# TigreGotico/phoonnx

Hardware: AMD Instinct MI355X
Metric: audio samples/sec (22.05 kHz), batch-32 256-phoneme utterances (higher is better)
Workload: dtype f32 (f16x3 split: fp32 operands as two fp16 planes, three MFMA products, fp32 accumulate)

## Files before the change

include/vitsmi.h:

```cpp
#ifndef VITSMI_H
#define VITSMI_H

#include <stddef.h>
#include <stdint.h>

#ifdef __cplusplus
extern "C" {
#endif

typedef struct vits_handle vits_handle;

enum {
    VITS_OK = 0,
    VITS_E_IO = -1,
    VITS_E_FORMAT = -2,
    VITS_E_ARG = -3,
    VITS_E_DEVICE = -4,
    VITS_E_NOMEM = -5,
    VITS_E_RANGE = -6
};

#define VITS_MAX_DIMS 4


// ... 418 lines not shown
    int res_planes;
    float res_slope;
    const float *old_out;
    const float *bias_b;
    int bias_b_stride;
    float div, oslope, oslope2, islope;
    const int64_t *lens;
    int rag_add, rag_mul;
    float sentinel;
    float *out;
    float *planes_out;
    float *res_seen;
    char kernel[128];
    int pack_cfg, run_cfg_used, rawin, s16, ck;
    float peak;
} vits_test_conv_sx_epi_args;
int vits_test_conv1d_sx_epi(int device_id, vits_test_conv_sx_epi_args *a);
int vits_test_conv1d_sx_planar(int device_id, const float *x, int B, int Cin, int T, const float *w, const float *bias,
                               int Cout, int K, int dil, int flags, const int64_t *lens, const float *old, int row_split,
                               int pl_rows, float *out, float *planes_out);
long long vits_test_set_sx_small_max(long long wgs);
int vits_test_conv1d_sx_gate(int device_id, const float *x, int B, int Cin, int T, const float *w, const float *bias,
                             const float *bias_b, int Cout, int K, int dil, int flags, float *out);
int vits_test_conv_transpose1d_sx(int device_id, const float *x, int B, int Cin, int T, const float *w,
                                  const float *bias, int Cout, int K, int stride, float *out);
int vits_bench_conv1d_sx(int device_id, int B, int Cin, int Cout, int T, int K, int dil, int dbg, int iters,
                         float *ms_out);
int vits_test_conv_pair_sx(int device_id, const float *x, int B, int C, int T, const float *w1, const float *b1,
                           const float *w2, const float *b2, int K, int dil1, int dil2, int chain, float slope, float *out,
                           float *ms_out);
// ... 1 lines not shown
typedef struct {
    int B, C, T, K, dil1, dil2, chain;
    int flags;
    float slope, div;
    const float *x;
    const float *w1, *b1, *w2, *b2;
    const int64_t *lens;
    const float *out_init;
    float *out;
    char kernel[128];
    int BNo;
} vits_test_conv_pair_sx_epi_args;
int vits_test_conv_pair_sx_epi(int device_id, vits_test_conv_pair_sx_epi_args *a);
int vits_test_split_identity(const float *x, int64_t n, uint16_t *h1_old, uint16_t *h1_fused);
int64_t vits_test_split_identity_sweep(uint32_t first, uint64_t count, uint32_t *first_bad);
int vits_test_split_forms(int device_id, const float *x, int n, float slope, int form, uint16_t *h0, uint16_t *h1, float *pk,
                          float *rec);
enum { VITS_P16_EPI_ACC = 1, VITS_P16_EPI_DIV = 2, VITS_P16_EPI_RAW = 4, VITS_P16_EPI_PLANES = 8 };
typedef struct {
    int B, C, T, K, dil1, dil2, chain;
    int precision;
    int flags;
    float slope, div, sentinel;
    const float *x;
    const float *w1, *b1, *w2, *b2;
    const float *old_out;
    const float *x_tail;
    const int64_t *lens;
    int rag_add, rag_mul;
    float *out;
// ... 139 lines not shown
```

phoonnx_amd/_ffi.py:

```python
import ctypes as C
import os

import numpy as np

from . import audio_encoding

_HERE = os.path.dirname(os.path.abspath(__file__))
_LIB = None

VITS_MAX_DIMS = 4


class VitsNoise(C.Structure):
    _fields_ = [("noise_dp", C.c_void_p), ("noise_z", C.c_void_p), ("noise_z_stride", C.c_int64),
                ("seed", C.c_uint64)]


class VitsOutput(C.Structure):
    _fields_ = [("data", C.POINTER(C.c_float)), ("dims", C.c_int64 * 4), ("y_lengths", C.POINTER(C.c_int64))]


class VitsStats(C.Structure):
    _fields_ = [("conv_flops", C.c_double), ("conv_bytes", C.c_double), ("dec_flops", C.c_double),
                ("dec_bytes", C.c_double), ("flow_flops", C.c_double), ("enc_flops", C.c_double),
# ... 15 lines not shown
               [(n, C.c_void_p) for n in ("x", "w", "bias", "lens", "bias_b")] + [("bias_b_stride", C.c_int), ("res", C.c_void_p)] + \
               [(n, C.c_int) for n in ("x_cstride", "out_cstride", "out_rows", "out_row0")] + \
               [("old_out", C.c_void_p), ("old_out2", C.c_void_p), ("sentinel", C.c_float), ("out", C.c_void_p), ("out2", C.c_void_p),
                ("pl_rows", C.c_int), ("planes_out", C.c_void_p), ("kernel", C.c_char * 128), ("cfg_used", C.c_int), ("ck_used", C.c_int)]


class VitsTestConvSxEpiArgs(C.Structure):
    _fields_ = [(n, C.c_int) for n in ("B", "Cin", "T", "Cout", "K", "dil", "pad_l", "stride", "precision", "force16", "no_s16",
                                       "min_cfg", "run_cfg", "flags")] + \
               [(n, C.c_void_p) for n in ("x", "w", "bias", "res")] + \
               [("res_is_x", C.c_int), ("res_planes", C.c_int), ("res_slope", C.c_float), ("old_out", C.c_void_p),
                ("bias_b", C.c_void_p), ("bias_b_stride", C.c_int)] + \
               [(n, C.c_float) for n in ("div", "oslope", "oslope2", "islope")] + \
               [("lens", C.c_void_p), ("rag_add", C.c_int), ("rag_mul", C.c_int), ("sentinel", C.c_float), ("out", C.c_void_p),
                ("planes_out", C.c_void_p), ("res_seen", C.c_void_p), ("kernel", C.c_char * 128)] + \
               [(n, C.c_int) for n in ("pack_cfg", "run_cfg_used", "rawin", "s16", "ck")] + [("peak", C.c_float)]


class VitsTestConvPair16EpiArgs(C.Structure):
    _fields_ = [(n, C.c_int) for n in ("B", "C", "T", "K", "dil1", "dil2", "chain", "precision", "flags")] + \
               [(n, C.c_float) for n in ("slope", "div", "sentinel")] + \
               [(n, C.c_void_p) for n in ("x", "w1", "b1", "w2", "b2", "old_out", "x_tail", "lens")] + \
               [("rag_add", C.c_int), ("rag_mul", C.c_int)] + \
               [(n, C.c_void_p) for n in ("out", "planes_out", "x_seen", "ms_out")] + [("kernel", C.c_char * 128)] + \
               [(n, C.c_int) for n in ("BN", "BNo", "ovl")] + [("peak", C.c_float), ("guard_ok", C.c_int)]


class VitsTestConvPairSxEpiArgs(C.Structure):
    _fields_ = [(n, C.c_int) for n in ("B", "C", "T", "K", "dil1", "dil2", "chain", "flags")] + \
               [(n, C.c_float) for n in ("slope", "div")] + \
               [(n, C.c_void_p) for n in ("x", "w1", "b1", "w2", "b2", "lens", "out_init", "out")] + \
# ... 133 lines not shown
    "vits_test_durations", "vits_test_expand_prior", "vits_test_fill_normal", "vits_test_fill_normal_rows", "vits_test_post_conv",
    "vits_delivery_plan", "vits_deliver", "vits_test_deliver",
    "vits_trim_range", "vits_delivery_plan_trimmed", "vits_deliver_trimmed", "vits_test_deliver_trimmed",
    "vits_loudness_filter", "vits_loudness_gate", "vits_level_gain", "vits_delivery_plan_leveled", "vits_deliver_leveled",
    "vits_test_loudness_blocks", "vits_test_deliver_leveled",
    "vits_shape_check", "vits_shape_gain", "vits_deliver_shaped", "vits_test_deliver_shaped",
    "vits_limit_check", "vits_limit_gains", "vits_deliver_limited", "vits_test_deliver_limited",
    "vits_run_chunked_enc", "vits_run_vocoder_chunked_enc", "vits_test_stream_pack",
    "vits_stream_shaping_check", "vits_stream_emit_range", "vits_run_chunked_enc_shaped", "vits_run_vocoder_chunked_enc_shaped",
    "vits_test_stream_pack_shaped",
    "vits_stream_onset_check", "vits_stream_onset_start", "vits_run_chunked_enc_trimmed", "vits_run_vocoder_chunked_enc_trimmed",
    "vits_test_stream_pack_trimmed",
    "vits_test_layernorm", "vits_test_dds", "vits_test_cf_pre", "vits_test_rqs_inverse", "vits_test_ea_logw",
    "vits_test_conv1d_epi", "vits_test_wn_gate", "vits_test_cond_matvec", "vits_test_conv1d_sx_epi",
    "vits_test_conv_pair16_epi", "vits_test_attention_form", "vits_test_conv_pair_sx_epi", "vits_test_split_forms", "vits_test_split_identity", "vits_test_split_identity_sweep",
]


G2P_EXPORTS = ["g2p_open", "g2p_close", "g2p_last_error", "g2p_hparam", "g2p_num_outputs", "g2p_output_name", "g2p_bucket",
               "g2p_run", "g2p_generate", "g2p_generate_batch", "g2p_test_forced_steps", "g2p_test_linear", "g2p_test_step"]


def lib_path():
    return os.environ.get("VITSMI_LIB") or os.path.join(_HERE, "libvitsmi.so")


def load():
    global _LIB
    if _LIB is not None:
        return _LIB
# ... 194 lines not shown
    lib.vits_test_conv1d_sx.argtypes = lib.vits_test_conv1d.argtypes
    lib.vits_test_conv_transpose1d_sx.argtypes = lib.vits_test_conv_transpose1d.argtypes
    lib.vits_test_conv1d_sx_planar.argtypes = [C.c_int, vp, C.c_int, C.c_int, C.c_int, vp, vp, C.c_int, C.c_int, C.c_int, C.c_int,
                                               vp, vp, C.c_int, C.c_int, vp, vp]
    lib.vits_test_set_sx_small_max.argtypes = [C.c_longlong]
    lib.vits_test_set_sx_small_max.restype = C.c_longlong
    lib.vits_test_conv1d_sx_gate.argtypes = [C.c_int, vp, C.c_int, C.c_int, C.c_int, vp, vp, vp, C.c_int, C.c_int, C.c_int, C.c_int, vp]
    lib.vits_bench_conv1d_sx.argtypes = [C.c_int] * 9 + [f32p]
    lib.vits_test_conv1d_epi.argtypes = [C.c_int, C.POINTER(VitsTestConvEpiArgs)]
    lib.vits_test_conv1d_sx_epi.argtypes = [C.c_int, C.POINTER(VitsTestConvSxEpiArgs)]
    lib.vits_test_conv_pair16_epi.argtypes = [C.c_int, C.POINTER(VitsTestConvPair16EpiArgs)]
    lib.vits_test_conv_pair_sx_epi.argtypes = [C.c_int, C.POINTER(VitsTestConvPairSxEpiArgs)]
    lib.vits_test_split_identity.argtypes = [vp, C.c_int64, vp, vp]
    lib.vits_test_split_identity_sweep.argtypes = [C.c_uint32, C.c_uint64, C.POINTER(C.c_uint32)]
    lib.vits_test_split_identity_sweep.restype = C.c_int64
    lib.vits_test_split_forms.argtypes = [C.c_int, vp, C.c_int, C.c_float, C.c_int, vp, vp, vp, vp]
    lib.vits_test_attention_form.argtypes = [C.c_int, C.POINTER(VitsTestAttentionFormArgs)]
    lib.vits_test_wn_gate.argtypes = [C.c_int, vp, C.c_int, C.c_int, C.c_int, C.c_int, vp]
    lib.vits_test_cond_matvec.argtypes = [C.c_int, vp, C.c_int, C.c_int, vp, C.c_int, vp, vp, C.c_int, vp]
    lib.vits_test_conv_pair_sx.argtypes = [C.c_int, vp, C.c_int, C.c_int, C.c_int, vp, vp, vp, vp, C.c_int, C.c_int,
                                           C.c_int, C.c_int, C.c_float, vp, f32p]
    lib.g2p_open.argtypes = [C.c_char_p, C.c_int, C.POINTER(vp)]
    lib.g2p_close.argtypes = [vp]
    lib.g2p_close.restype = None
    lib.g2p_last_error.argtypes = [vp]
    lib.g2p_last_error.restype = C.c_char_p
    lib.g2p_hparam.argtypes = [vp, C.c_char_p, i64p]
    lib.g2p_num_outputs.argtypes = [vp]
    lib.g2p_output_name.argtypes = [vp, C.c_int]
    lib.g2p_output_name.restype = C.c_char_p
# ... 18 lines not shown
```

phoonnx_amd/csrc/conv_sx_engine.hip.hpp:

```cpp
#pragma once
#include <hip/hip_runtime.h>
#include <stdint.h>

#include <cstdio>
#include <cstdlib>
#include <string>
#include <utility>

#include "conv_engine.hip.hpp"
#include "conv_geom.hpp"

#ifndef SX_CFG0_WIDE
#define SX_CFG0_WIDE 0
#endif
#ifndef SX16_SPREAD
#define SX16_SPREAD 0
#endif
#ifndef SX16_PRIO
#define SX16_PRIO 0
#endif
#ifndef SX16_ABL
#define SX16_ABL 0
#endif
#ifndef SX16_NA_SMALL
#define SX16_NA_SMALL 2
#endif
#ifndef SX16_WIDE
#define SX16_WIDE 1
#endif
#ifndef SX_NOA
#define SX_NOA 0
#endif
#ifndef SX_XCD_GROUP_DEFAULT
#define SX_XCD_GROUP_DEFAULT 4
#endif
namespace vitsmi {

typedef __bf16 bf16x8 __attribute__((ext_vector_type(8)));
typedef _Float16 f16x8 __attribute__((ext_vector_type(8)));

enum : int { SX_NO_RAW_STORE = 256 };

struct SxRagged {
    const int *len;
    int add, mul;
};
// ... 33 lines not shown
    int64_t planar_bstride;
    int RS;
    int s16;
    unsigned magic;
    unsigned x_bytes;
    unsigned lds_bytes;
    int NT, MT, B;
    int flags;
    float div, oslope, oslope2;
    float wscale;
    unsigned long long *prof;
    unsigned *peak;
    SxRagged rag;
    int zt_p = -1;
    int xgs = 0;
};

inline int sx_xcd_group_shift() {
    static const int v = [] {
        const char *e = std::getenv("VITSMI_XCD_GROUP");
        int g = e ? std::atoi(e) : SX_XCD_GROUP_DEFAULT, s = 0;
        while ((2 << s) <= g && s < 4) s++;
        return s;
    }();
    return v;
}
__device__ __forceinline__ int sx_xcd_tile(int tseq, int xcd, int xgs) {
    return ((tseq >> xgs) << (xgs + 3)) + (xcd << xgs) + (tseq & ((1 << xgs) - 1));
}

// ... 88 lines not shown
}

__device__ __forceinline__ float f16_bits_to_f32(unsigned short h) { return (float)__builtin_bit_cast(_Float16, h); }

enum : int {
    SX_HAS_RAW = 1 << 9,
    SX_HAS_PL = 1 << 10,
    SX_RAW_ACT = 1 << 11,
    SX_PL_ACT = 1 << 12,
    SX_HAS_BIASB = 1 << 13,
    SX_RES_EARLY = 1 << 14,
    SX_GATE = 1 << 15,
    SX_WN_RMW = 1 << 19,
    SX_PLANAR_STORE2 = 1 << 20,
    SX_PLANAR_COUPLING = 1 << 21,
    SX_RES_PL = 1 << 22
};
constexpr int kSxEpiMask = EPI_RES | EPI_ACC | EPI_DIV | SX_HAS_RAW | SX_HAS_PL | SX_RAW_ACT | SX_PL_ACT | SX_HAS_BIASB | SX_RES_EARLY |
                           SX_GATE | SX_RES_PL;

template <int MW, int NW, int WM, int WN, int EPI = -1, bool PROF = false, bool RAWIN = false, int NP = 6, int SH = 32>
__global__ __launch_bounds__(256, (MW * NW > 8) ? 1 : ((SH == 16 && MW * NW == 2 && !RAWIN) ? 3 : 2)) void conv_sx_kernel(SxArgs a) {
    constexpr int BM = MW * WM * 32, BN = NW * WN * 32, MB = BM / 32;
    constexpr bool S16 = SH == 16;
    static_assert(SH == 32 || (SH == 16 && (NP == 2 || NP == 1) && !RAWIN && !PROF), "16x16x32: fp16 arithmetics on plane inputs");
    static_assert(NP == 6 || NP == 1 || NP == 2, "arithmetic");
    static_assert(NP != 1 || SH == 16, "the single-plane mode exists on the 16x16x32 loop only");
    constexpr bool H1 = NP == 1;
    constexpr bool F16 = NP == 2 || H1;
    constexpr int NPROD = H1 ? 1 : (F16 ? 3 : NP);
    constexpr int NPL = NP == 6 ? 3 : (H1 ? 1 : 2);
// ... 737 lines not shown
    const float *resb = a.res + (int64_t)b * a.raw_bstride;
    const uint16_t *resplb = a.res_pl + (int64_t)b * a.pl_bstride;
    const float unsl = a.res_unslope;
    const bool respl = H1 || (EPI >= 0 ? (EPI & SX_RES_PL) != 0 : a.res_pl != nullptr);
    const bool res_epi = (flags & EPI_RES) && !PRE;
    const float *addp = res_epi ? resb : rawb;
    const bool has_add = res_epi || (flags & EPI_ACC);
    const bool two_adds = res_epi && (flags & EPI_ACC);
    const float oslope = a.oslope, oslope2 = a.oslope2, rdiv = a.div;
    const float wsc = a.wscale;
    const int64_t plane_elems = (int64_t)CGo * Tout * 8;
    const float *biasp = a.bias ? a.bias : a.zeros;
    const int b_on = a.bias ? 1 : 0;
    constexpr int NRND = MW * (NW / 2);
    constexpr bool PIPE = EPI >= 0 && ((EPI & EPI_RES) != 0 && !PRE) != ((EPI & EPI_ACC) != 0);
    f32x4 adb[PIPE ? 2 : 1][2][4], ad2[2][4];
    auto geom = [&](int m, int n, int &co0, int &r, int &t) {
        const int row0 = mt * BM + (wm * MW + m) * 32;
        r = u == 1 ? 0 : (row0 >> 5) % u;
        co0 = u == 1 ? row0 : (row0 / (32 * u)) * 32;
        t = t0 + (wn * NW + n) * 32 + l31;
    };
    auto cell_at = [&](int co0, int r, int t, int q) -> int64_t {
        return ((int64_t)((co0 >> 3) + q) * Tout + (t * u + r)) * 8 + 4 * hi;
    };
    auto issue_adds = [&](auto R, auto P) {
        constexpr int rr = decltype(R)::value, pp = decltype(P)::value;
        constexpr int m = rr / (NW / 2), n0 = (rr % (NW / 2)) * 2;
#pragma unroll
        for (int j = 0; j < 2; j++) {
            int co0, r, t;
            geom(m, n0 + j, co0, r, t);
            const int tl = t < T ? t : T - 1;
#pragma unroll
            for (int q = 0; q < 4; q++) {
                const int64_t c = cell_at(co0, r, tl, q);
                if (respl) {
                    if (res_epi) {
                        float o4[4];
                        if constexpr (H1) {
                            unact4h(*reinterpret_cast<const u32x2 *>(resplb + c), unsl, o4);
                        } else {
                            float h0[4], h1[4];
                            unact4h(*reinterpret_cast<const u32x2 *>(resplb + c), 1.f, h0);
                            unact4h(*reinterpret_cast<const u32x2 *>(resplb + plane_elems + c), 1.f, h1);
#pragma unroll
                            for (int e = 0; e < 4; e++) {
// ... 24 lines not shown
        const int row0 = mt * BM + (wm * MW + m) * 32;
        f32x4 bq[4];
#pragma unroll
        for (int q = 0; q < 4; q++) {
            bq[q] = *reinterpret_cast<const f32x4 *>(biasp + (row0 + 8 * q + 4 * hi) * b_on);
            if (flags & SX_HAS_BIASB)
                bq[q] += *reinterpret_cast<const f32x4 *>(a.bias_b + (int64_t)b * a.bias_b_stride + co0m + 8 * q + 4 * hi);
        }
#pragma unroll
        for (int j = 0; j < 2; j++) {
            constexpr int dummy = 0;
            (void)dummy;
            const int n = n0 + j;
            int co0, r, t;
            geom(m, n, co0, r, t);
            if (t >= TV) continue;
#pragma unroll
            for (int q = 0; q < 4; q++) {
                const int64_t cell = cell_at(co0, r, t, q);
                f32x4 v;
#pragma unroll
                for (int e = 0; e < 4; e++) {
                    if constexpr (F16) v[e] = __builtin_fmaf(acc[m][n][4 * q + e], wsc, bq[q][e]);
                    else v[e] = acc[m][n][4 * q + e] + bq[q][e];
                }
                if constexpr (PRE) v += pre[rr][j][q];
                if (has_add) v += adb[pp][j][q];
                if (two_adds) v += ad2[j][q];
                if (flags & EPI_DIV) {
#pragma unroll
                    for (int e = 0; e < 4; e++) v[e] = v[e] / rdiv;
                }
                if (flags & SX_HAS_RAW) {
                    f32x4 o = v;
                    if (flags & SX_RAW_ACT) {
#pragma unroll
                        for (int e = 0; e < 4; e++) o[e] = fmaxf(v[e], v[e] * oslope);
                    }
                    *reinterpret_cast<f32x4 *>(rawb + cell) = o;
                }
                if (flags & SX_HAS_PL) {
                    f32x4 o = v;
                    if (flags & SX_PL_ACT) {
#pragma unroll
                        for (int e = 0; e < 4; e++) o[e] = fmaxf(v[e], v[e] * oslope2);
                    }
                    unsigned wa[3], wb[3];
                    if constexpr (H1) {
                        wa[0] = cvt1h_pair_pk(o[0], o[1], pk);
                        wb[0] = cvt1h_pair_pk(o[2], o[3], pk);
                    } else if constexpr (F16) {
                        split2h_pair_pk(o[0], o[1], wa[0], wa[1], pk);
                        split2h_pair_pk(o[2], o[3], wb[0], wb[1], pk);
                    } else {
                        split3_pair(o[0], o[1], wa[0], wa[1], wa[2]);
                        split3_pair(o[2], o[3], wb[0], wb[1], wb[2]);
                    }
#pragma unroll
                    for (int pl = 0; pl < NPL; pl++)
                        *reinterpret_cast<u32x2 *>(plb + pl * plane_elems + cell) = u32x2{wa[pl], wb[pl]};
                }
            }
        }
    });
    if constexpr (F16) {
        if (a.peak) {
            if constexpr (S16) sx_publish_peak_at(a.peak, (int)blockIdx.x, pk, reinterpret_cast<float *>(lds_sx));
            else sx_publish_peak(a.peak, (int)blockIdx.x, pk);
        }
    }
}


template <int MW, int NW, int WM, int WN, int EPI = -1, bool PROF = false, bool RAWIN = false, int NP = 6, int SH = 32>
inline hipError_t launch_conv_sx_k(const SxArgs &a, dim3 grid, size_t lds, hipStream_t stream) {
    static std::atomic<uint64_t> attr_done{0};
    auto kern = conv_sx_kernel<MW, NW, WM, WN, EPI, PROF, RAWIN, NP, SH>;
    if (hipError_t e = sx_allow_big_lds(reinterpret_cast<const void *>(kern), attr_done); e != hipSuccess) return e;
    if (g_launch_name_on)
// ... 82 lines not shown
    if (!g.fits) return hipErrorInvalidValue;
    a.LW = g.LW;
    a.RS = g.RS;
    a.magic = (unsigned)((0x100000000ull + a.RS - 1) / a.RS);
    a.x_bytes = g.x_bytes;
    const size_t lds = g.lds;
    a.lds_bytes = (unsigned)lds;
    if (s16 && ((long long)(2 * (a.Cin / 8) + 2) * a.T) * 16 >= (1ll << 32)) return hipErrorInvalidValue;
    if (rawin && (cfg == 0 || !g.raw_ok || !a.xr || (long long)a.T * 64 + 64 >= (1ll << 32))) return hipErrorInvalidValue;
    if (a.oslope == 0.f) a.oslope = 1.f;
    if (a.oslope2 == 0.f) a.oslope2 = 1.f;
    if (a.islope == 0.f) a.islope = 1.f;
    if (a.Cin % 16 || a.Cout % 32 || a.Cr % 32 || a.Cout % BM) return hipErrorInvalidValue;
    a.NT = (a.T + BN - 1) / BN;
    a.MT = a.Cout / BM;
    a.B = B;
    const long long nb = (long long)a.NT * B;
    if (nb == 0) return hipSuccess;
    a.xgs = a.NT >= (2 << sx_xcd_group_shift()) ? sx_xcd_group_shift() : 0;
    const long long per_round = 8ll << a.xgs;
    const long long wgs = (nb + per_round - 1) / per_round * per_round * a.MT;
    if (wgs >= (1ll << 31)) return hipErrorInvalidValue;
    dim3 grid((unsigned)wgs, 1, 1);
    int epi = a.flags & (EPI_RES | EPI_ACC | EPI_DIV);
    if (a.out_raw && !(a.flags & SX_NO_RAW_STORE)) epi |= SX_HAS_RAW | (a.oslope != 1.f ? SX_RAW_ACT : 0);
    if (a.out_pl && !(a.flags & SX_GATE)) epi |= SX_HAS_PL | (a.oslope2 != 1.f ? SX_PL_ACT : 0);
    if (a.bias_b) epi |= SX_HAS_BIASB;
    if (a.res_pl && nprod == 2 && (a.flags & EPI_RES)) {
        if (a.res || rawin || (a.flags & (SX_WN_RMW | SX_GATE))) return hipErrorInvalidValue;
        epi |= SX_RES_PL;
// ... 211 lines not shown
```

phoonnx_amd/csrc/sx_split.hip.hpp:

```cpp
#pragma once
#include <hip/hip_runtime.h>
#include <stdint.h>

#include <atomic>

#include "conv_geom.hpp"

namespace vitsmi {

typedef float sxf32x2 __attribute__((ext_vector_type(2)));
typedef _Float16 f16x2 __attribute__((ext_vector_type(2)));
typedef unsigned u32x4 __attribute__((ext_vector_type(4)));
typedef unsigned u32x2 __attribute__((ext_vector_type(2)));

constexpr int kSxPeakSlots = 64;
constexpr float kF16Max = 65504.f;

inline thread_local bool g_launch_name_on = false;
inline thread_local char g_launch_name[128];

__device__ __forceinline__ unsigned cvt_pk_f16(float lo, float hi) {
    const sxf32x2 v = {lo, hi};
    return __builtin_bit_cast(unsigned, __builtin_convertvector(v, f16x2));
}
// ... 36 lines not shown
    float r;
    asm("v_max_f32 %0, %1, %2" : "=v"(r) : "v"(x), "v"(m));
    return r;
}
__device__ __forceinline__ unsigned cvt1h_pair_pk(float x, float y, float &pk) {
    pk = __builtin_fmaxf(pk, __builtin_fmaxf(__builtin_fabsf(x), __builtin_fabsf(y)));
    return cvt_pk_f16(__builtin_amdgcn_fmed3f(x, -65504.f, 65504.f), __builtin_amdgcn_fmed3f(y, -65504.f, 65504.f));
}
__device__ __forceinline__ void unact4h(u32x2 w, float unslope, float (&o)[4]) {
    const unsigned wx = w.x, wy = w.y;
    const f16x2 a = __builtin_bit_cast(f16x2, wx), b = __builtin_bit_cast(f16x2, wy);
    const float v[4] = {(float)a[0], (float)a[1], (float)b[0], (float)b[1]};
#pragma unroll
    for (int e = 0; e < 4; e++) o[e] = v[e] < 0.f ? v[e] * unslope : v[e];
}

constexpr int kSxPeakStride = 32;
inline hipError_t sx_allow_big_lds(const void *kern, std::atomic<uint64_t> &done) {
    int dev = 0;
    if (hipGetDevice(&dev) != hipSuccess) return hipGetLastError();
    const uint64_t bit = 1ull << (dev & 63);
    if (done.load(std::memory_order_acquire) & bit) return hipSuccess;
    const hipError_t e = hipFuncSetAttribute(kern, hipFuncAttributeMaxDynamicSharedMemorySize, kSxMaxDynLds);
    if (e == hipSuccess) done.fetch_or(bit, std::memory_order_release);
    return e;
}
__device__ __forceinline__ void sx_publish_peak_at(unsigned *slots, int slot_idx, float pk, float *s_pk) {
#pragma unroll
    for (int o = 32; o > 0; o >>= 1) pk = __builtin_fmaxf(pk, __shfl_xor(pk, o, 64));
    __syncthreads();
// ... 41 lines not shown
```

phoonnx_amd/csrc/vitsmi.hip:

```cpp
#include <climits>
#include <hip/hip_runtime.h>

#include <cmath>
#include <cstdarg>
#include <chrono>
#include <cstdio>
#include <cstring>
#include <mutex>
#include <string>
#include <vector>

#include "../../include/vitsmi.h"
#include "conv_geom.hpp"
#include "conv_sx_engine.hip.hpp"
#include "conv_sx_pair.hip.hpp"
#include "conv_sx_pair16.hip.hpp"
#include "attention16.hip.hpp"
#include "conv_sx_small.hip.hpp"
#include "delivery.hip.hpp"
#include "delivery_run.hip.hpp"
#include "fit.hip.hpp"
#include "shape.hip.hpp"
#include "kernels.hip.hpp"
#include "loudness.hip.hpp"
// ... 4569 lines not shown
    if (dres) sx_block_kernel<<<gout, 256>>>(dresin, (int64_t)Cr * To, To, nullptr, dres, Cr, To);
    if (dresp) sx_split_planes_kernel<<<gout, 256>>>(dresin, (int64_t)Cr * To, To, nullptr, dresp, Cr, To, mode);
    TCHECK(hipGetLastError());
    SxArgs a = sx_args(d, dA, dA, T);
    a.xp = reinterpret_cast<const u32x4 *>(dxp);
    a.xr = dxr;
    a.islope = p->islope;
    a.bias_b = dbb;
    a.bias_b_stride = p->bias_b_stride;
    a.out_raw = draw;
    a.out_pl = dop;
    a.res = p->res_is_x ? dxr : dres;
    a.res_pl = dresp;
    a.res_unslope = p->res_planes ? 1.f / p->res_slope : 1.f;
    a.flags = (f_res ? EPI_RES : 0) | (f_acc ? EPI_ACC : 0) | ((flags & VITS_SX_EPI_DIV) ? EPI_DIV : 0) |
              ((flags & VITS_SX_EPI_NO_RAW_STORE) ? SX_NO_RAW_STORE : 0);
    a.div = p->div == 0.f ? 1.f : p->div;
    a.oslope = p->oslope;
    a.oslope2 = p->oslope2;
    a.rag = SxRagged{dlen, p->rag_add, p->rag_mul};
    a.peak = dpk;
    const bool name_was_on = g_launch_name_on;
    g_launch_name_on = true;
    g_launch_name[0] = 0;
    const hipError_t le = launch_conv_sx(a, run, B, nullptr, d.rawin, nprod, d.cfg);
    g_launch_name_on = name_was_on;
    if (le != hipSuccess) return fail(nullptr, VITS_E_DEVICE, "sx conv epilogue hook: launch_conv_sx: %s", hipGetErrorString(le));
    std::snprintf(p->kernel, sizeof p->kernel, "%s", g_launch_name);
    p->pack_cfg = d.cfg;
    p->run_cfg_used = run;
    p->rawin = d.rawin ? 1 : 0;
// ... 432 lines not shown
int64_t vits_test_split_identity_sweep(uint32_t first, uint64_t count, uint32_t *first_bad) {
    int64_t bad = 0;
    for (uint64_t k = 0; k < count; k++) {
        const uint32_t bits = first + (uint32_t)k;
        uint16_t o, f;
        split_identity_one(__builtin_bit_cast(float, bits), &o, &f);
        const bool nan_o = (o & 0x7fffu) > 0x7c00u, nan_f = (f & 0x7fffu) > 0x7c00u;
        if (o != f && !(nan_o && nan_f)) {
            if (bad == 0 && first_bad) *first_bad = bits;
            bad++;
        }
    }
    return bad;
}

int vits_test_split_forms(int device_id, const float *x, int n, float slope, int form, uint16_t *h0, uint16_t *h1, float *pk, float *rec) {
    if (int rc = test_dev(device_id)) return rc;
    if (!x || n < 2 || (n & 1) || !(slope > 0.f) || slope > 1.f || form < 0 || form > 1 || !h0 || !h1 || !pk || !rec)
        return fail(nullptr, VITS_E_ARG, "split forms hook: n even and >= 2, 0 < slope <= 1, form 0 or 1, every output given");
    DevBufs D;
    float *dx = D.up(x, (size_t)n);
    uint16_t *d0 = D.alloc<uint16_t>((size_t)n), *d1 = D.alloc<uint16_t>((size_t)n);
    float *dpk = D.alloc<float>((size_t)n / 2), *drec = D.alloc<float>((size_t)n);
    TCHECK(D.err);
    const unsigned blocks = (unsigned)((n / 2 + 255) / 256);
    if (form == 0) split_forms_kernel<0><<<blocks, 256>>>(dx, n, slope, 1.f / slope, d0, d1, dpk, drec);
    else split_forms_kernel<1><<<blocks, 256>>>(dx, n, slope, 1.f / slope, d0, d1, dpk, drec);
    TCHECK(hipGetLastError());
    TCHECK(hipDeviceSynchronize());
    TCHECK(download(h0, d0, (size_t)n));
// ... 1274 lines not shown
```

phoonnx_amd/session.py:

```python
import contextlib
import ctypes as C
import dataclasses
import time
from collections import namedtuple
from dataclasses import dataclass
from typing import Dict, List, Optional, Sequence

import numpy as np

from . import _ffi


class SessionError(RuntimeError):
    """Raised for every failure of the engine (onnxruntime raises its own
    InvalidArgument/RuntimeException at voice.py:374; callers there do not catch either)."""


class RangeError(SessionError):
    """VITS_E_RANGE: the f16x3 generator arithmetic met an activation beyond the range of its fp16 operand planes
    (|x| > 65504) or a non-finite value.  The engine reports this instead of returning clamped audio; `MiSession`
    (range_fallback=True, the default) then reopens the voice with the bf16x6 arithmetic (fp32 range) and repeats the
    call, so user code only sees this when the fallback is switched off or impossible (borrowed weight arena)."""


# ... 2183 lines not shown
    a.old_out, a.old_out2, a.sentinel = _ffi.ptr(old_out), _ffi.ptr(old_out2), CONV_EPI_SENTINEL
    a.out, a.out2, a.pl_rows, a.planes_out = _ffi.ptr(out), _ffi.ptr(o2), pl_rows, _ffi.ptr(pl)
    rc = lib.vits_test_conv1d_epi(device_id, C.byref(a))
    if rc != 0:
        raise SessionError(_ffi.last_error(None))
    return {"out": out, "out2": o2, "planes": pl, "kernel": a.kernel.decode(), "cfg": a.cfg_used, "ck": a.ck_used}


SX_EPI_FLAGS = {"res": 1, "acc": 2, "div": 4, "no_raw_store": 8}
SX_PRECISIONS = {"bf16x6": 0, "f16x3": 1, "f16": 2}


def test_conv1d_sx_epi(x, w, bias=None, flags=(), precision="f16x3", dil=1, pad_l=None, stride=1, force16=False, no_s16=False,
                       min_cfg=0, run_cfg=-1, res=None, res_is_x=False, res_planes=False, res_slope=1.0, old_out=None,
                       bias_b=None, div=1.0, oslope=1.0, oslope2=1.0, islope=1.0, raw=True, planes=False, lens=None,
                       rag_add=0, rag_mul=1, sentinel=CONV_EPI_SENTINEL, device_id=0):
    lib = _ffi.load()
    f32 = lambda a: None if a is None else np.ascontiguousarray(a, np.float32)
    x, w, bias, bias_b, res, old_out = (f32(a) for a in (x, w, bias, bias_b, res, old_out))
    B, Cin, T = x.shape
    Cout, K = (w.shape[1] if stride > 1 else w.shape[0]), w.shape[2]
    To = T * stride
    ln = None if lens is None else np.ascontiguousarray(lens, np.int64)
    for name, arr, shape in (("w", w, (Cin, Cout, K) if stride > 1 else (Cout, Cin, K)), ("bias", bias, (Cout,)),
                             ("res", res, (B, Cout, To)), ("old_out", old_out, (B, Cout, To)), ("lens", ln, (B,))):
        if arr is not None and arr.shape != shape:
            raise ValueError(f"{name} has shape {arr.shape}, the launch needs {shape}")
    if bias_b is not None and (bias_b.ndim != 2 or bias_b.shape[0] != B):
        raise ValueError(f"bias_b has shape {bias_b.shape}, the launch needs ({B}, stride)")
    out = np.empty((B, Cout, To), np.float32) if raw else None
    pl = np.empty((B, Cout, To), np.float32) if planes else None
    seen = np.empty((B, Cout, To), np.float32) if (res_planes and res is not None) else None
    a = _ffi.VitsTestConvSxEpiArgs()
    a.B, a.Cin, a.T, a.Cout, a.K, a.dil, a.stride = B, Cin, T, Cout, K, dil, stride
    a.pad_l = dil * (K - 1) // 2 if pad_l is None else pad_l
    a.precision, a.force16, a.no_s16, a.min_cfg, a.run_cfg = SX_PRECISIONS[precision], int(force16), int(no_s16), min_cfg, run_cfg
    a.flags = sum(SX_EPI_FLAGS[f] for f in flags)
    a.x, a.w, a.bias, a.res, a.old_out, a.bias_b, a.lens = (_ffi.ptr(v) for v in (x, w, bias, res, old_out, bias_b, ln))
    a.res_is_x, a.res_planes, a.res_slope = int(res_is_x), int(res_planes), res_slope
    a.bias_b_stride = 0 if bias_b is None else bias_b.shape[1]
    a.div, a.oslope, a.oslope2, a.islope = div, oslope, oslope2, islope
    a.rag_add, a.rag_mul, a.sentinel = rag_add, rag_mul, sentinel
    a.out, a.planes_out, a.res_seen = _ffi.ptr(out), _ffi.ptr(pl), _ffi.ptr(seen)
    rc = lib.vits_test_conv1d_sx_epi(device_id, C.byref(a))
    if rc != 0:
        raise SessionError(_ffi.last_error(None))
    return {"out": out, "planes": pl, "res_seen": seen, "kernel": a.kernel.decode(), "pack_cfg": a.pack_cfg, "run_cfg": a.run_cfg_used,
            "rawin": bool(a.rawin), "s16": bool(a.s16), "ck": a.ck, "peak": float(a.peak)}


def test_wn_gate(a, blocked=False, device_id=0):
    lib = _ffi.load()
    a = np.ascontiguousarray(a, np.float32)
    B, C2, T = a.shape
    if C2 % 2:
        raise ValueError("a holds the tanh rows and as many sigmoid rows")
    out = np.empty((B, C2 // 2, T), np.float32)
# ... 79 lines not shown
    out = np.empty((B, Cc, T), np.float32)
    pl = np.empty((B, Cc, T), np.float32) if "planes" in flags else None
    seen = np.empty((B, Cc, T), np.float32)
    a = _ffi.VitsTestConvPair16EpiArgs()
    a.B, a.C, a.T, a.K, a.dil1, a.dil2, a.chain = B, Cc, T, K, dil1, dil2, int(bool(chain))
    a.precision, a.flags = SX_PRECISIONS[precision], sum(P16_EPI_FLAGS[f] for f in flags)
    a.slope, a.div, a.sentinel = slope, div, sentinel
    a.x, a.w1, a.b1, a.w2, a.b2, a.old_out, a.x_tail, a.lens = (_ffi.ptr(v) for v in (x, w1, b1, w2, b2, old_out, x_tail, ln))
    a.rag_add, a.rag_mul = rag_add, rag_mul
    a.out, a.planes_out, a.x_seen = _ffi.ptr(out), _ffi.ptr(pl), _ffi.ptr(seen)
    rc = lib.vits_test_conv_pair16_epi(device_id, C.byref(a))
    if rc != 0:
        raise SessionError(_ffi.last_error(None))
    return {"out": out, "planes": pl, "x_seen": seen, "kernel": a.kernel.decode(), "BN": a.BN, "BNo": a.BNo, "ovl": bool(a.ovl),
            "peak": float(a.peak), "guard_ok": bool(a.guard_ok)}


def test_split_forms(x, slope=0.1, form="pair", device_id=0):
    lib = _ffi.load()
    x = np.ascontiguousarray(x, np.float32)
    if x.ndim != 1 or x.size < 2 or x.size % 2:
        raise ValueError("x: one dimension, an even number of values")
    n = x.size
    h0, h1 = np.empty(n, np.uint16), np.empty(n, np.uint16)
    pk, rec = np.empty(n // 2, np.float32), np.empty(n, np.float32)
    rc = lib.vits_test_split_forms(device_id, _ffi.ptr(x), n, float(slope), {"engine": 0, "pair": 1}[form], _ffi.ptr(h0), _ffi.ptr(h1),
                                   _ffi.ptr(pk), _ffi.ptr(rec))
    if rc != 0:
        raise SessionError(_ffi.last_error(None))
    return {"h0": h0.view(np.float16), "h1": h1.view(np.float16), "pk": pk, "rec": rec}
# ... 929 lines not shown
```

Baseline: 139.7 million.

## Add interior-tile fast path to sx conv epilogue with 32-bit addressing and mixed ops

Splits the sx conv epilogue into an interior variant, used when the whole time tile lies inside the valid length, and the existing edge variant. The interior path skips per-column bounds clamping, computes addresses with a 32-bit lane offset and a magic-number division in place of a modulo, and uses v_fma_mix/v_min and mixed split helpers for the residual un-activation and plane splitting. A host-side guard forces the edge path when 32-bit offsets could overflow or the unslope identity does not hold. This adds code size and register pressure from instantiating the epilogue twice.

```diff
diff --git a/include/vitsmi.h b/include/vitsmi.h
--- a/include/vitsmi.h
+++ b/include/vitsmi.h
@@ -456,6 +456,7 @@
     char kernel[128];
     int pack_cfg, run_cfg_used, rawin, s16, ck;
     float peak;
+    int force_edge;
 } vits_test_conv_sx_epi_args;
 int vits_test_conv1d_sx_epi(int device_id, vits_test_conv_sx_epi_args *a);
 int vits_test_conv1d_sx_planar(int device_id, const float *x, int B, int Cin, int T, const float *w, const float *bias,
@@ -487,6 +488,8 @@
 int vits_test_conv_pair_sx_epi(int device_id, vits_test_conv_pair_sx_epi_args *a);
 int vits_test_split_identity(const float *x, int64_t n, uint16_t *h1_old, uint16_t *h1_fused);
 int64_t vits_test_split_identity_sweep(uint32_t first, uint64_t count, uint32_t *first_bad);
+int64_t vits_test_unact_identity_sweep(uint32_t first, uint64_t count, float unslope, uint32_t *first_bad);
+int64_t vits_test_unact_identity_sweep_dev(int device_id, float unslope, uint32_t *first_bad);
 int vits_test_split_forms(int device_id, const float *x, int n, float slope, int form, uint16_t *h0, uint16_t *h1, float *pk,
                           float *rec);
 enum { VITS_P16_EPI_ACC = 1, VITS_P16_EPI_DIV = 2, VITS_P16_EPI_RAW = 4, VITS_P16_EPI_PLANES = 8 };
diff --git a/phoonnx_amd/_ffi.py b/phoonnx_amd/_ffi.py
--- a/phoonnx_amd/_ffi.py
+++ b/phoonnx_amd/_ffi.py
@@ -53,7 +53,7 @@
                [(n, C.c_float) for n in ("div", "oslope", "oslope2", "islope")] + \
                [("lens", C.c_void_p), ("rag_add", C.c_int), ("rag_mul", C.c_int), ("sentinel", C.c_float), ("out", C.c_void_p),
                 ("planes_out", C.c_void_p), ("res_seen", C.c_void_p), ("kernel", C.c_char * 128)] + \
-               [(n, C.c_int) for n in ("pack_cfg", "run_cfg_used", "rawin", "s16", "ck")] + [("peak", C.c_float)]
+               [(n, C.c_int) for n in ("pack_cfg", "run_cfg_used", "rawin", "s16", "ck")] + [("peak", C.c_float), ("force_edge", C.c_int)]
 
 
 class VitsTestConvPair16EpiArgs(C.Structure):
@@ -217,6 +217,7 @@
     "vits_test_layernorm", "vits_test_dds", "vits_test_cf_pre", "vits_test_rqs_inverse", "vits_test_ea_logw",
     "vits_test_conv1d_epi", "vits_test_wn_gate", "vits_test_cond_matvec", "vits_test_conv1d_sx_epi",
     "vits_test_conv_pair16_epi", "vits_test_attention_form", "vits_test_conv_pair_sx_epi", "vits_test_split_forms", "vits_test_split_identity", "vits_test_split_identity_sweep",
+    "vits_test_unact_identity_sweep", "vits_test_unact_identity_sweep_dev",
 ]
 
 
@@ -441,6 +442,10 @@
     lib.vits_test_split_identity.argtypes = [vp, C.c_int64, vp, vp]
     lib.vits_test_split_identity_sweep.argtypes = [C.c_uint32, C.c_uint64, C.POINTER(C.c_uint32)]
     lib.vits_test_split_identity_sweep.restype = C.c_int64
+    lib.vits_test_unact_identity_sweep.argtypes = [C.c_uint32, C.c_uint64, C.c_float, C.POINTER(C.c_uint32)]
+    lib.vits_test_unact_identity_sweep.restype = C.c_int64
+    lib.vits_test_unact_identity_sweep_dev.argtypes = [C.c_int, C.c_float, C.POINTER(C.c_uint32)]
+    lib.vits_test_unact_identity_sweep_dev.restype = C.c_int64
     lib.vits_test_split_forms.argtypes = [C.c_int, vp, C.c_int, C.c_float, C.c_int, vp, vp, vp, vp]
     lib.vits_test_attention_form.argtypes = [C.c_int, C.POINTER(VitsTestAttentionFormArgs)]
     lib.vits_test_wn_gate.argtypes = [C.c_int, vp, C.c_int, C.c_int, C.c_int, C.c_int, vp]
diff --git a/phoonnx_amd/csrc/conv_sx_engine.hip.hpp b/phoonnx_amd/csrc/conv_sx_engine.hip.hpp
--- a/phoonnx_amd/csrc/conv_sx_engine.hip.hpp
+++ b/phoonnx_amd/csrc/conv_sx_engine.hip.hpp
@@ -30,6 +30,18 @@
 #endif
 #ifndef SX_NOA
 #define SX_NOA 0
+#endif
+#ifndef SX_EPI_INTERIOR
+#define SX_EPI_INTERIOR 1
+#endif
+#ifndef SX_EPI_ADDR32
+#define SX_EPI_ADDR32 1
+#endif
+#ifndef SX_EPI_MIX
+#define SX_EPI_MIX 1
+#endif
+#ifndef SX_EPI_RESMIX
+#define SX_EPI_RESMIX 1
 #endif
 #ifndef SX_XCD_GROUP_DEFAULT
 #define SX_XCD_GROUP_DEFAULT 4
@@ -93,6 +105,7 @@
     SxRagged rag;
     int zt_p = -1;
     int xgs = 0;
+    unsigned umagic = 1u << 31;
 };
 
 inline int sx_xcd_group_shift() {
@@ -211,7 +224,8 @@
     SX_WN_RMW = 1 << 19,
     SX_PLANAR_STORE2 = 1 << 20,
     SX_PLANAR_COUPLING = 1 << 21,
-    SX_RES_PL = 1 << 22
+    SX_RES_PL = 1 << 22,
+    SX_FORCE_EDGE = 1 << 23
 };
 constexpr int kSxEpiMask = EPI_RES | EPI_ACC | EPI_DIV | SX_HAS_RAW | SX_HAS_PL | SX_RAW_ACT | SX_PL_ACT | SX_HAS_BIASB | SX_RES_EARLY |
                            SX_GATE | SX_RES_PL;
@@ -979,9 +993,25 @@
     const int b_on = a.bias ? 1 : 0;
     constexpr int NRND = MW * (NW / 2);
     constexpr bool PIPE = EPI >= 0 && ((EPI & EPI_RES) != 0 && !PRE) != ((EPI & EPI_ACC) != 0);
+    constexpr bool HAS_INTR = SX_EPI_INTERIOR != 0 && NP == 2 && !RAWIN && EPI >= 0;
+    auto epilogue = [&](auto INTR_) __attribute__((always_inline)) {
+    constexpr bool INTR = decltype(INTR_)::value;
+    constexpr bool A32 = INTR && SX_EPI_ADDR32 != 0;
+    constexpr bool MIX = INTR && SX_EPI_MIX != 0;
     f32x4 adb[PIPE ? 2 : 1][2][4], ad2[2][4];
+    const uint32_t lane32 = ((uint32_t)(t0 + wn * NW * 32 + l31) * (uint32_t)u) * 32u + 16u * (uint32_t)hi;
+    auto row_at = [&](int co0, int r, int n, int q) -> int64_t {
+        return ((int64_t)((co0 >> 3) + q) * Tout + (n * 32 * u + r)) * 8;
+    };
     auto geom = [&](int m, int n, int &co0, int &r, int &t) {
         const int row0 = mt * BM + (wm * MW + m) * 32;
+        if constexpr (A32) {
+            const int blk = row0 >> 5, qd = (int)(((uint64_t)(uint32_t)blk * a.umagic) >> 31);
+            r = blk - qd * u;
+            co0 = qd * 32;
+            t = t0 + (wn * NW + n) * 32 + l31;
+            return;
+        }
         r = u == 1 ? 0 : (row0 >> 5) % u;
         co0 = u == 1 ? row0 : (row0 / (32 * u)) * 32;
         t = t0 + (wn * NW + n) * 32 + l31;
@@ -996,6 +1026,27 @@
         for (int j = 0; j < 2; j++) {
             int co0, r, t;
             geom(m, n0 + j, co0, r, t);
+            if constexpr (INTR) {
+#pragma unroll
+                for (int q = 0; q < 4; q++) {
+                    const int64_t c = A32 ? row_at(co0, r, n0 + j, q) : cell_at(co0, r, t, q);
+                    const uint32_t o4b = A32 ? lane32 : 0u, o2b = A32 ? lane32 >> 1 : 0u;
+                    const auto f4 = [&](const float *p) { return *reinterpret_cast<const f32x4 *>(reinterpret_cast<const char *>(p + c) + o4b); };
+                    const auto h4 = [&](const uint16_t *p) { return *reinterpret_cast<const u32x2 *>(reinterpret_cast<const char *>(p + c) + o2b); };
+                    if (respl) {
+                        if (res_epi) {
+                            float o4[4];
+                            if constexpr (SX_EPI_RESMIX != 0) unact4h_planes_mix(h4(resplb), h4(resplb + plane_elems), unsl, o4);
+                            else unact4h_planes(h4(resplb), h4(resplb + plane_elems), unsl, o4);
+                            adb[pp][j][q] = f32x4{o4[0], o4[1], o4[2], o4[3]};
+                        } else if (has_add)
+                            adb[pp][j][q] = f4(rawb);
+                    } else if (has_add)
+                        adb[pp][j][q] = f4(addp);
+                    if (two_adds) ad2[j][q] = f4(rawb);
+                }
+                continue;
+            }
             const int tl = t < T ? t : T - 1;
 #pragma unroll
             for (int q = 0; q < 4; q++) {
@@ -1050,10 +1101,13 @@
             const int n = n0 + j;
             int co0, r, t;
             geom(m, n, co0, r, t);
-            if (t >= TV) continue;
+            if constexpr (!INTR) {
+                if (t >= TV) continue;
+            }
 #pragma unroll
             for (int q = 0; q < 4; q++) {
-                const int64_t cell = cell_at(co0, r, t, q);
+                const int64_t cell = A32 ? row_at(co0, r, n, q) : cell_at(co0, r, t, q);
+                const uint32_t o4b = A32 ? lane32 : 0u, o2b = A32 ? lane32 >> 1 : 0u;
                 f32x4 v;
 #pragma unroll
                 for (int e = 0; e < 4; e++) {
@@ -1071,20 +1125,23 @@
                     f32x4 o = v;
                     if (flags & SX_RAW_ACT) {
 #pragma unroll
-                        for (int e = 0; e < 4; e++) o[e] = fmaxf(v[e], v[e] * oslope);
+                        for (int e = 0; e < 4; e++) o[e] = MIX ? lrelu_max(v[e], oslope) : fmaxf(v[e], v[e] * oslope);
                     }
-                    *reinterpret_cast<f32x4 *>(rawb + cell) = o;
+                    *reinterpret_cast<f32x4 *>(reinterpret_cast<char *>(rawb + cell) + o4b) = o;
                 }
                 if (flags & SX_HAS_PL) {
                     f32x4 o = v;
                     if (flags & SX_PL_ACT) {
 #pragma unroll
-                        for (int e = 0; e < 4; e++) o[e] = fmaxf(v[e], v[e] * oslope2);
+                        for (int e = 0; e < 4; e++) o[e] = MIX ? lrelu_max(v[e], oslope2) : fmaxf(v[e], v[e] * oslope2);
                     }
                     unsigned wa[3], wb[3];
                     if constexpr (H1) {
                         wa[0] = cvt1h_pair_pk(o[0], o[1], pk);
                         wb[0] = cvt1h_pair_pk(o[2], o[3], pk);
+                    } else if constexpr (MIX) {
+                        split2h_pair_pk_mix(o[0], o[1], wa[0], wa[1], pk);
+                        split2h_pair_pk_mix(o[2], o[3], wb[0], wb[1], pk);
                     } else if constexpr (F16) {
                         split2h_pair_pk(o[0], o[1], wa[0], wa[1], pk);
                         split2h_pair_pk(o[2], o[3], wb[0], wb[1], pk);
@@ -1094,11 +1151,17 @@
                     }
 #pragma unroll
                     for (int pl = 0; pl < NPL; pl++)
-                        *reinterpret_cast<u32x2 *>(plb + pl * plane_elems + cell) = u32x2{wa[pl], wb[pl]};
+                        *reinterpret_cast<u32x2 *>(reinterpret_cast<char *>(plb + pl * plane_elems + cell) + o2b) = u32x2{wa[pl], wb[pl]};
                 }
             }
         }
     });
+    };
+    if constexpr (HAS_INTR) {
+        if (SX_EPI_INTERIOR == 2 || (t0 + BN <= TV && !(a.flags & SX_FORCE_EDGE))) epilogue(std::true_type{});
+        else epilogue(std::false_type{});
+    } else
+        epilogue(std::false_type{});
     if constexpr (F16) {
         if (a.peak) {
             if constexpr (S16) sx_publish_peak_at(a.peak, (int)blockIdx.x, pk, reinterpret_cast<float *>(lds_sx));
@@ -1211,6 +1274,10 @@
     if (a.Cin % 16 || a.Cout % 32 || a.Cr % 32 || a.Cout % BM) return hipErrorInvalidValue;
     a.NT = (a.T + BN - 1) / BN;
     a.MT = a.Cout / BM;
+    a.umagic = a.ups > 1 ? (unsigned)(((1ull << 31) + a.ups - 1) / a.ups) : 1u << 31;
+    if (a.ups < 1 || (long long)a.T * a.ups * 32 + 64 >= (1ll << 32) || (long long)(a.Cout / 32) * a.ups >= (1ll << 31) ||
+        (a.res_pl && a.res_unslope != 0.f && !(a.res_unslope >= 1.f)))
+        a.flags |= SX_FORCE_EDGE;
     a.B = B;
     const long long nb = (long long)a.NT * B;
     if (nb == 0) return hipSuccess;
diff --git a/phoonnx_amd/csrc/sx_split.hip.hpp b/phoonnx_amd/csrc/sx_split.hip.hpp
--- a/phoonnx_amd/csrc/sx_split.hip.hpp
+++ b/phoonnx_amd/csrc/sx_split.hip.hpp
@@ -74,6 +74,29 @@
 #pragma unroll
     for (int e = 0; e < 4; e++) o[e] = v[e] < 0.f ? v[e] * unslope : v[e];
 }
+__device__ __forceinline__ void unact4h_planes_mix(u32x2 w0, u32x2 w1, float unslope, float (&o)[4]) {
+    const unsigned a[2] = {w0.x, w0.y}, b[2] = {w1.x, w1.y};
+    const float c = 1.f / 2048.f;
+#pragma unroll
+    for (int k = 0; k < 2; k++) {
+        float lo, hi;
+        asm("v_fma_mix_f32 %0, %1, %2, %3 op_sel_hi:[1,0,1]" : "=v"(lo) : "v"(b[k]), "v"(c), "v"(a[k]));
+        asm("v_fma_mix_f32 %0, %1, %2, %3 op_sel:[1,0,1] op_sel_hi:[1,0,1]" : "=v"(hi) : "v"(b[k]), "v"(c), "v"(a[k]));
+        const float ml = lo * unslope, mh = hi * unslope;
+        asm("v_min_f32 %0, %1, %2" : "=v"(o[2 * k]) : "v"(lo), "v"(ml));
+        asm("v_min_f32 %0, %1, %2" : "=v"(o[2 * k + 1]) : "v"(hi), "v"(mh));
+    }
+}
+__device__ __forceinline__ void unact4h_planes(u32x2 w0, u32x2 w1, float unslope, float (&o)[4]) {
+    float h0[4], h1[4];
+    unact4h(w0, 1.f, h0);
+    unact4h(w1, 1.f, h1);
+#pragma unroll
+    for (int e = 0; e < 4; e++) {
+        const float v = __builtin_fmaf(h1[e], 1.f / 2048.f, h0[e]);
+        o[e] = v < 0.f ? v * unslope : v;
+    }
+}
 
 constexpr int kSxPeakStride = 32;
 inline hipError_t sx_allow_big_lds(const void *kern, std::atomic<uint64_t> &done) {
diff --git a/phoonnx_amd/csrc/vitsmi.hip b/phoonnx_amd/csrc/vitsmi.hip
--- a/phoonnx_amd/csrc/vitsmi.hip
+++ b/phoonnx_amd/csrc/vitsmi.hip
@@ -4607,7 +4607,7 @@
     a.res_pl = dresp;
     a.res_unslope = p->res_planes ? 1.f / p->res_slope : 1.f;
     a.flags = (f_res ? EPI_RES : 0) | (f_acc ? EPI_ACC : 0) | ((flags & VITS_SX_EPI_DIV) ? EPI_DIV : 0) |
-              ((flags & VITS_SX_EPI_NO_RAW_STORE) ? SX_NO_RAW_STORE : 0);
+              ((flags & VITS_SX_EPI_NO_RAW_STORE) ? SX_NO_RAW_STORE : 0) | (p->force_edge ? SX_FORCE_EDGE : 0);
     a.div = p->div == 0.f ? 1.f : p->div;
     a.oslope = p->oslope;
     a.oslope2 = p->oslope2;
@@ -5070,6 +5070,40 @@
     return bad;
 }
 
+int64_t vits_test_unact_identity_sweep(uint32_t first, uint64_t count, float unslope, uint32_t *first_bad) {
+    if (!(unslope >= 1.f)) return fail(nullptr, VITS_E_ARG, "unact identity: unslope >= 1");
+    int64_t bad = 0;
+    for (uint64_t k = 0; k < count; k++) {
+        const uint32_t p = first + (uint32_t)k;
+        const float h0 = (float)__builtin_bit_cast(_Float16, (uint16_t)(p & 0xffffu));
+        const float h1 = (float)__builtin_bit_cast(_Float16, (uint16_t)(p >> 16));
+        const float v = std::fmaf(h1, 1.f / 2048.f, h0);
+        const float o = v < 0.f ? v * unslope : v, n = std::fmin(v, v * unslope);
+        if (__builtin_bit_cast(uint32_t, o) != __builtin_bit_cast(uint32_t, n) && !(o != o && n != n)) {
+            if (bad == 0 && first_bad) *first_bad = p;
+            bad++;
+        }
+    }
+    return bad;
+}
+int64_t vits_test_unact_identity_sweep_dev(int device_id, float unslope, uint32_t *first_bad) {
+    if (int rc = test_dev(device_id)) return rc;
+    if (!(unslope >= 1.f)) return fail(nullptr, VITS_E_ARG, "unact identity: unslope >= 1");
+    DevBufs D;
+    unsigned long long *dcount = D.fill<unsigned long long>(1);
+    unsigned *dfirst = D.fill<unsigned>(1, 0xff);
+    TCHECK(D.err);
+    unact_identity_sweep_kernel<<<65536, 256>>>(unslope, dcount, dfirst);
+    TCHECK(hipGetLastError());
+    TCHECK(hipDeviceSynchronize());
+    unsigned long long count = 0;
+    unsigned fb = 0;
+    TCHECK(download(&count, dcount, 1));
+    TCHECK(download(&fb, dfirst, 1));
+    if (first_bad && count) *first_bad = fb;
+    return (int64_t)count;
+}
+
 int vits_test_split_forms(int device_id, const float *x, int n, float slope, int form, uint16_t *h0, uint16_t *h1, float *pk, float *rec) {
     if (int rc = test_dev(device_id)) return rc;
     if (!x || n < 2 || (n & 1) || !(slope > 0.f) || slope > 1.f || form < 0 || form > 1 || !h0 || !h1 || !pk || !rec)
diff --git a/phoonnx_amd/session.py b/phoonnx_amd/session.py
--- a/phoonnx_amd/session.py
+++ b/phoonnx_amd/session.py
@@ -2221,7 +2221,7 @@
 def test_conv1d_sx_epi(x, w, bias=None, flags=(), precision="f16x3", dil=1, pad_l=None, stride=1, force16=False, no_s16=False,
                        min_cfg=0, run_cfg=-1, res=None, res_is_x=False, res_planes=False, res_slope=1.0, old_out=None,
                        bias_b=None, div=1.0, oslope=1.0, oslope2=1.0, islope=1.0, raw=True, planes=False, lens=None,
-                       rag_add=0, rag_mul=1, sentinel=CONV_EPI_SENTINEL, device_id=0):
+                       rag_add=0, rag_mul=1, sentinel=CONV_EPI_SENTINEL, force_edge=False, device_id=0):
     lib = _ffi.load()
     f32 = lambda a: None if a is None else np.ascontiguousarray(a, np.float32)
     x, w, bias, bias_b, res, old_out = (f32(a) for a in (x, w, bias, bias_b, res, old_out))
@@ -2247,7 +2247,7 @@
     a.res_is_x, a.res_planes, a.res_slope = int(res_is_x), int(res_planes), res_slope
     a.bias_b_stride = 0 if bias_b is None else bias_b.shape[1]
     a.div, a.oslope, a.oslope2, a.islope = div, oslope, oslope2, islope
-    a.rag_add, a.rag_mul, a.sentinel = rag_add, rag_mul, sentinel
+    a.rag_add, a.rag_mul, a.sentinel, a.force_edge = rag_add, rag_mul, sentinel, int(force_edge)
     a.out, a.planes_out, a.res_seen = _ffi.ptr(out), _ffi.ptr(pl), _ffi.ptr(seen)
     rc = lib.vits_test_conv1d_sx_epi(device_id, C.byref(a))
     if rc != 0:
@@ -2357,6 +2357,15 @@
         raise SessionError(_ffi.last_error(None))
     return {"out": out, "planes": pl, "x_seen": seen, "kernel": a.kernel.decode(), "BN": a.BN, "BNo": a.BNo, "ovl": bool(a.ovl),
             "peak": float(a.peak), "guard_ok": bool(a.guard_ok)}
+
+
+def test_unact_identity_sweep_dev(unslope, device_id=0):
+    lib = _ffi.load()
+    bad = C.c_uint32(0)
+    n = lib.vits_test_unact_identity_sweep_dev(device_id, float(unslope), C.byref(bad))
+    if n < 0:
+        raise SessionError(_ffi.last_error(None))
+    return int(n), int(bad.value)
 
 
 def test_split_forms(x, slope=0.1, form="pair", device_id=0):
```

Result: no change. 140.9 million (median of 6 runs) (+0.9%).
